# SeekStorm/SeekStorm

Measured on NVIDIA H100. Metric: queries/sec at top-10 (1M x 768 f32 cosine brute-force kNN), higher is better.
Workload: dtype f32

## Files before the change

seekstorm_b200/csrc/api.cu:

```cuda
#include <stdarg.h>
#include <string.h>
#include <algorithm>
#include <condition_variable>
#include <exception>
#include <memory>
#include <mutex>
#include <new>
#include <shared_mutex>
#include <vector>

#include "bm25.h"
#include "comm.h"
#include "common.cuh"
#include "vec_scan.h"

namespace ssb {

static thread_local char g_err[512] = "";

void set_error(const char* fmt, ...) {
    va_list ap; va_start(ap, fmt);
    vsnprintf(g_err, sizeof(g_err), fmt, ap);
    va_end(ap);
}
// ... 150 lines not shown
    const void* qsrc = queries;
    if (!is_device_ptr(queries)) {
        SSB_TRY(c.qstage.reserve(((size_t)nq * ix->dims + 3) / (queries_i8 ? 4 : 1) + 1, 0, st));
        SSB_CUDA_TRY(cudaMemcpyAsync(c.qstage.p, queries, qbytes, cudaMemcpyHostToDevice, st));
        c.stats.h2d_bytes += qbytes;
        qsrc = c.qstage.p;
    }
    if (scan == vec::Scan::I8_128) {
        SSB_TRY(c.q_i8.reserve((size_t)nq_pad * ix->dpad8, 0, st));
        if (queries_i8 && (ix->turbo || ix->cfg.vector_similarity != SSB_SIM_COSINE)) { set_error("int8 query codes are accepted for Cosine + ScalarQuantizationI8 only (the other quantisers need the query scale)"); return SSB_E_UNSUPPORTED; }
        if (ix->turbo) {
            SSB_TRY(c.q_scale.reserve(nq_pad, 0, st)); SSB_TRY(c.q_norm.reserve(nq_pad, 0, st));
            SSB_TRY(vec::launch_quantize_rows_turbo_i8((const float*)qsrc, ix->dims, nq, nq_pad, ix->dims, ix->tq_dim, ix->tq_mask, c.q_i8.p, ix->dpad8, c.q_scale.p,
                                                       c.q_norm.p, ix->cfg.vector_similarity == SSB_SIM_COSINE, ix->cfg.vector_similarity != SSB_SIM_EUCLIDEAN, st));
        } else if (ix->affine) {
            SSB_TRY(c.q_scale.reserve(nq_pad, 0, st)); SSB_TRY(c.q_norm.reserve(nq_pad, 0, st)); SSB_TRY(c.q_aff.reserve((size_t)nq_pad * 2, 0, st));
            SSB_TRY(vec::launch_quantize_rows_affine_i8((const float*)qsrc, ix->dims, nq, nq_pad, ix->dims, nullptr, nullptr, ix->aff_min, ix->aff_max, c.q_i8.p, ix->dpad8,
                                                        c.q_scale.p, c.q_norm.p, c.q_aff.p, 1, st));
        } else if (ix->cfg.vector_similarity != SSB_SIM_COSINE) {
            SSB_TRY(c.q_scale.reserve(nq_pad, 0, st)); SSB_TRY(c.q_norm.reserve(nq_pad, 0, st));
            SSB_TRY(vec::launch_quantize_rows_scale_i8((const float*)qsrc, ix->dims, nq, nq_pad, ix->dims, c.q_i8.p, ix->dpad8, c.q_scale.p, c.q_norm.p,
                                                       ix->cfg.vector_similarity == SSB_SIM_EUCLIDEAN, st));
        } else if (queries_i8) {
            SSB_CUDA_TRY(cudaMemsetAsync(c.q_i8.p, 0, (size_t)nq_pad * ix->dpad8, st));
            SSB_CUDA_TRY(cudaMemcpy2DAsync(c.q_i8.p, ix->dpad8, qsrc, ix->dims, ix->dims, nq, cudaMemcpyDeviceToDevice, st));
        } else {
            SSB_TRY(vec::launch_quantize_rows_i8((const float*)qsrc, ix->dims, nq, nq_pad, ix->dims, c.q_i8.p, ix->dpad8, st));
        }
    } else if (filter || scan == vec::Scan::Bf16_64 || scan == vec::Scan::Bf16_128 || scan == vec::Scan::Bf16_256) {
        SSB_TRY(c.qhi.reserve((size_t)nq_pad * ix->dpad, 0, st));
        SSB_TRY(c.qlo.reserve((size_t)nq_pad * ix->dpad, 0, st));
        if (filter) SSB_TRY(c.q_scale.reserve(nq_pad, 0, st));
        SSB_TRY(vec::launch_prep_split_queries_bf16((const float*)qsrc, nq, ix->dims, ix->dims, c.qhi.p, c.qlo.p, nq_pad, ix->dpad,
                                                    ix->cfg.vector_similarity == SSB_SIM_COSINE, st, (filter || ivf) ? c.qpad.p : nullptr,
                                                    filter ? c.q_scale.p : nullptr, filter ? ix->vec_err.p : nullptr));
    } else
    SSB_TRY(vec::launch_prep_queries((const float*)qsrc, nq, ix->dims, ix->dims, c.qpad.p, nq_pad, ix->dpad,
                                     ix->cfg.vector_similarity == SSB_SIM_COSINE, st));
    c.stats.kernel_launches += 1;
    if (ix->n_rows == 0) { SSB_CUDA_TRY(cudaMemsetAsync(keys_out_dev, 0, (size_t)nq * LIST * 8, st)); return SSB_OK; }
    size_t sb = vec::is_tensor_core(scan) ? vec::scan_tc_scratch_bytes(ix->n_sms, nq_pad) : vec::scan_scratch_bytes(ix->n_sms, nq_pad);
    const size_t head_words = sb / 8 + (size_t)nq_pad * LIST + (nq_pad + 1) / 2;
    SSB_TRY(c.scratch.reserve(head_words + (filter ? vec::refine_scratch_words(ix->n_sms, nq_pad) : 0), 0, st));
    vec::ScanArgs a{};
    a.rows = ix->rows.p; a.rows_hi = ix->rows_hi.p; a.rows_lo = ix->rows_lo.p; a.rows_h16 = ix->rows_h16.p; a.doc_ids = ix->doc_ids.p; a.n_rows = ix->n_rows; a.dpad = ix->dpad; a.queries_padded = c.qpad.p;
    a.nq_pad = nq_pad; a.nq_valid = nq; a.k = k; a.similarity = ix->cfg.vector_similarity; a.n_sms = ix->n_sms;
    a.scratch = c.scratch.p; a.scratch_bytes = sb;
    uint64_t* merged = c.scratch.p + sb / 8;
    a.keys_out = merged; a.ev0 = c.ev0; a.ev1 = c.ev1; c.ev_used = true;
    a.thr_buf = reinterpret_cast<uint32_t*>(merged + (size_t)nq_pad * LIST);
    a.ceil_keys = ceil_dev;
    if (ix->del.n) { a.del_slot = ix->del.d_slot; a.del_words = ix->del.d_words; }
    a.launches = &c.stats.kernel_launches;
    if (ivf) {
        vec::IvfArgs v{};
        v.medoids = ix->medoids.p; v.lvl_begin = ix->lvl_begin.p; v.cl_count = ix->cl_count.p;
        v.n_clusters = ix->n_clusters; v.n_levels = (uint32_t)ix->h_lvl_begin.size(); v.max_level_clusters = ix->max_level_clusters;
        v.queries_padded = c.qpad.p; v.nq = nq; v.nq_pad = nq_pad; v.dpad = ix->dpad; v.similarity = ix->cfg.vector_similarity;
        v.ann_mode = ivf->mode; v.n_probe = ivf->n_probe; v.cluster_threshold = ivf->thr;
        v.words = (ix->n_clusters + 31) / 32;
        SSB_TRY(c.ivf_scores.reserve((size_t)nq * ix->n_clusters, 0, st));
        SSB_TRY(c.ivf_sel.reserve((size_t)nq_pad * v.words, 0, st));
        SSB_TRY(c.ivf_obs.reserve(nq, 0, st));
        v.scores = c.ivf_scores.p; v.sel = c.ivf_sel.p; v.observed = c.ivf_obs.p; v.launches = &c.stats.kernel_launches;
        SSB_TRY(vec::launch_ivf_select(v, st));
        a.ivf_sel = c.ivf_sel.p; a.ivf_words = v.words; a.row_cluster = ix->row_cluster.p;
    }
    if (scan == vec::Scan::I8_128) {
        a.rows_i8 = ix->rows_i8.p; a.queries_i8 = c.q_i8.p; a.dpad8 = ix->dpad8;
        if (ix->turbo || ix->cfg.vector_similarity != SSB_SIM_COSINE) {
            a.i8_scaled = ix->cfg.vector_similarity == SSB_SIM_EUCLIDEAN ? (ix->affine ? 3 : 2) : 1;
            a.row_aff = ix->row_aff.p; a.q_aff = c.q_aff.p;
            a.row_scale = ix->row_scale.p; a.row_norm = ix->row_norm.p; a.q_scale = c.q_scale.p; a.q_norm = c.q_norm.p;
        }
    } else if (vec::is_tensor_core(scan)) {
        SSB_TRY(c.qhi.reserve((size_t)nq_pad * ix->dpad, 0, st));
        SSB_TRY(c.qlo.reserve((size_t)nq_pad * ix->dpad, 0, st));
        a.q_hi = c.qhi.p; a.q_lo = c.qlo.p;
        if (filter) a.q_scale = c.q_scale.p;
    }
    SSB_TRY(vec::is_tensor_core(scan) ? vec::launch_scan_tc(a, scan, st) : vec::launch_scan_ffma(a, st));
    if (filter) {
        vec::RefineArgs r{};
        r.rows = ix->rows.p; r.doc_ids = ix->doc_ids.p; r.n_rows = ix->n_rows; r.dpad = ix->dpad; r.queries_padded = c.qpad.p; r.margin = c.q_scale.p;
        r.keys = merged; r.keys_out = keys_out_dev;
        r.nq = nq; r.nq_pad = nq_pad; r.k = k;
        r.fb_lists = c.scratch.p + head_words;
        r.fb_state = reinterpret_cast<uint32_t*>(r.fb_lists + (size_t)nq_pad * ix->n_sms * LIST);
        r.del_slot = a.del_slot; r.del_words = a.del_words; r.ivf_sel = a.ivf_sel; r.ivf_words = a.ivf_words; r.row_cluster = a.row_cluster; r.n_sms = ix->n_sms; r.launches = &c.stats.kernel_launches;
        SSB_TRY(vec::launch_refine(r, st));
        c.fb_state = r.fb_state;
    } else {
        SSB_CUDA_TRY(cudaMemcpyAsync(keys_out_dev, merged, (size_t)nq * LIST * 8, cudaMemcpyDeviceToDevice, st));
    }
    const uint64_t pass_bytes = ix->n_rows * ix->dims * (scan == vec::Scan::I8_128 ? 1 : 4);
    c.stats.algorithmic_bytes += passes * pass_bytes;
    c.stats.scan_bytes_read += filter ? passes * pass_bytes / 2 + (uint64_t)nq * LIST * ix->dims * 4 : passes * pass_bytes;
    return SSB_OK;
}

uint32_t decode_list(const uint64_t* keys, uint32_t k, ssb_hit* hits, bool dedup) {
    uint32_t n = 0;
    for (uint32_t j = 0; j < LIST && n < k; j++) {
        const uint64_t key = keys[j];
        if (!key) break;
        const uint64_t doc = key_doc(key);
        if (dedup) { bool seen = false; for (uint32_t i = 0; i < n; i++) seen = seen || hits[i].doc_id == doc; if (seen) continue; }
        hits[n].doc_id = doc; hits[n].score = key_score(key); hits[n].pad = 0;
        n++;
    }
    return n;
}

void decode_keys(const uint64_t* keys, uint32_t nq, uint32_t k, ssb_hit* hits, uint32_t* n_hits, bool dedup = false) {
    for (uint32_t q = 0; q < nq; q++) {
        const uint32_t n = decode_list(keys + (size_t)q * LIST, k, hits + (size_t)q * k, dedup);
        for (uint32_t j = n; j < k; j++) { hits[(size_t)q * k + j].doc_id = 0; hits[(size_t)q * k + j].score = 0.f; hits[(size_t)q * k + j].pad = 0; }
        if (n_hits) n_hits[q] = n;
    }
}

int32_t shard_merge(ssb_index* ix, SearchCtx& c, uint64_t* keys_dev, uint32_t nq) {
    if (!ix->comm.active() || nq == 0) return SSB_OK;
    const size_t n = (size_t)nq * LIST;
    SSB_TRY(c.gather.reserve(n * ix->comm.world, 0, c.st));
    SSB_TRY(comm_all_gather_u64(ix->comm, keys_dev, c.gather.p, n, c.st));
    SSB_TRY(vec::launch_merge_lists(c.gather.p, ix->comm.world, nq, keys_dev, c.st));
    c.stats.kernel_launches += 2;
    return SSB_OK;
}
int32_t shard_sum_counts(ssb_index* ix, SearchCtx& c, uint64_t* counts_dev, uint32_t nq) {
    if (!ix->comm.active() || nq == 0 || !counts_dev) return SSB_OK;
    SSB_TRY(comm_all_reduce_sum_u64(ix->comm, counts_dev, nq, c.st));
    c.stats.kernel_launches += 1;
    return SSB_OK;
}

template <int W>
// ... 1031 lines not shown
```

seekstorm_b200/csrc/common.cuh:

```cuda
#pragma once
#include <cuda_runtime.h>
#include <cuda.h>
#include <stdint.h>
#include <stdio.h>
#include <string>

#include "../../include/seekstorm_b200.h"

namespace ssb {

void set_error(const char* fmt, ...);

#define SSB_CUDA_TRY(expr)                                                                   \
    do {                                                                                     \
        cudaError_t _e = (expr);                                                             \
        if (_e != cudaSuccess) {                                                             \
            ssb::set_error("%s:%d CUDA error %d (%s) in %s", __FILE__, __LINE__, (int)_e,   \
                           cudaGetErrorString(_e), #expr);                                   \
            return _e == cudaErrorMemoryAllocation ? SSB_E_NOMEM : SSB_E_CUDA;               \
        }                                                                                    \
    } while (0)

#define SSB_TRY(expr)                      \
    do {                                   \
// ... 21 lines not shown
#endif
}
__host__ __device__ __forceinline__ uint64_t pack_key(float score, uint32_t doc) {
    return ((uint64_t)ord_f32(score) << 32) | (uint64_t)(0xFFFFFFFFu - doc);
}
__host__ __device__ __forceinline__ uint32_t key_doc(uint64_t k) { return 0xFFFFFFFFu - (uint32_t)k; }
__host__ __device__ __forceinline__ float key_score(uint64_t k) { return unord_f32((uint32_t)(k >> 32)); }

#ifdef __CUDACC__
__device__ __forceinline__ uint64_t shfl64(uint64_t v, int src) {
    uint32_t lo = __shfl_sync(FULL, (uint32_t)v, src), hi = __shfl_sync(FULL, (uint32_t)(v >> 32), src);
    return ((uint64_t)hi << 32) | lo;
}
__device__ __forceinline__ uint64_t shfl64_up1(uint64_t v) {
    uint32_t lo = __shfl_up_sync(FULL, (uint32_t)v, 1), hi = __shfl_up_sync(FULL, (uint32_t)(v >> 32), 1);
    return ((uint64_t)hi << 32) | lo;
}
__device__ __forceinline__ uint64_t shfl64_xor(uint64_t v, int m) {
    uint32_t lo = __shfl_xor_sync(FULL, (uint32_t)v, m), hi = __shfl_xor_sync(FULL, (uint32_t)(v >> 32), m);
    return ((uint64_t)hi << 32) | lo;
}
__device__ __forceinline__ void wl_insert(uint64_t& L, uint64_t cand, int lane) {
    unsigned gt = __ballot_sync(FULL, L >= cand);
    int pos = __popc(gt);
    if (__any_sync(FULL, L == cand)) return;
    uint64_t up = shfl64_up1(L);
    if (lane == pos) L = cand;
    else if (lane > pos) L = up;
}
__device__ __forceinline__ uint64_t wl_sort_desc(uint64_t v, int lane) {
#pragma unroll
    for (int k = 2; k <= 32; k <<= 1) {
#pragma unroll
        for (int j = k >> 1; j > 0; j >>= 1) {
            const uint64_t p = shfl64_xor(v, j);
            const bool keep_max = ((lane & k) == 0) == ((lane & j) == 0);
            v = keep_max ? (v > p ? v : p) : (v < p ? v : p);
        }
    }
    return v;
}
__device__ __forceinline__ uint64_t wl_merge(uint64_t A, uint64_t B, int lane) {
    uint64_t Br = shfl64(B, 31 - lane);
    uint64_t M = A > Br ? A : Br;
#pragma unroll
    for (int s = 16; s >= 1; s >>= 1) {
        uint64_t P = shfl64_xor(M, s);
        bool keep_max = (lane & s) == 0;
        M = keep_max ? (M > P ? M : P) : (M < P ? M : P);
    }
    return M;
}

__device__ __forceinline__ bool doc_deleted(const uint32_t* __restrict__ del_slot, const uint64_t* __restrict__ del_words, uint32_t doc) {
    if (!del_slot) return false;
    const uint32_t slot = __ldg(&del_slot[doc >> 16]);
    if (slot == 0xFFFFFFFFu) return false;
    return ((__ldg(&del_words[(size_t)slot * 1024 + ((doc & 0xFFFFu) >> 6)]) >> (doc & 63u)) & 1ull) != 0;
}

__device__ __forceinline__ bool ivf_skipped(const uint32_t* __restrict__ sel, uint32_t words, uint32_t q, const uint32_t* __restrict__ row_cluster, uint32_t row) {
    if (!sel) return false;
    const uint32_t c = __ldg(&row_cluster[row]);
    return ((__ldg(&sel[(size_t)q * words + (c >> 5)]) >> (c & 31u)) & 1u) == 0u;
}

__device__ __forceinline__ uint32_t smem_u32(const void* p) { return (uint32_t)__cvta_generic_to_shared(p); }

__device__ __forceinline__ void mbar_init(uint64_t* bar, uint32_t count) {
    asm volatile("mbarrier.init.shared::cta.b64 [%0], %1;" ::"r"(smem_u32(bar)), "r"(count));
}
__device__ __forceinline__ void fence_mbar_init() {
    asm volatile("fence.mbarrier_init.release.cluster;" ::: "memory");
}
__device__ __forceinline__ void fence_proxy_async() {
    asm volatile("fence.proxy.async.shared::cta;" ::: "memory");
}
__device__ __forceinline__ void mbar_arrive_expect_tx(uint64_t* bar, uint32_t bytes) {
    asm volatile("mbarrier.arrive.expect_tx.shared::cta.b64 _, [%0], %1;" ::"r"(smem_u32(bar)), "r"(bytes)
                 : "memory");
}
__device__ __forceinline__ void mbar_arrive(uint64_t* bar) {
    asm volatile("mbarrier.arrive.shared::cta.b64 _, [%0];" ::"r"(smem_u32(bar)) : "memory");
}
__device__ __forceinline__ void mbar_wait(uint64_t* bar, uint32_t parity) {
    asm volatile(
        "{\n"
        ".reg .pred p;\n"
        "WAIT_LOOP:\n"
        "mbarrier.try_wait.parity.shared::cta.b64 p, [%0], %1;\n"
        "@p bra.uni WAIT_DONE;\n"
        "bra.uni WAIT_LOOP;\n"
        "WAIT_DONE:\n"
        "}\n" ::"r"(smem_u32(bar)),
        "r"(parity)
        : "memory");
}
__device__ __forceinline__ void tma_load_2d(void* dst, const CUtensorMap* map, int c0, int c1, uint64_t* bar) {
    asm volatile(
        "cp.async.bulk.tensor.2d.shared::cluster.global.mbarrier::complete_tx::bytes [%0], [%1, {%3, %4}], [%2];"
        ::"r"(smem_u32(dst)), "l"(map), "r"(smem_u32(bar)), "r"(c0), "r"(c1)
        : "memory");
}
__device__ __forceinline__ void tma_prefetch_desc(const CUtensorMap* map) {
    asm volatile("prefetch.tensormap [%0];" ::"l"(map) : "memory");
}
// ... 9 lines not shown
```

seekstorm_b200/csrc/vec_refine.cu:

```cuda
#include "common.cuh"
#include "vec_scan.h"

namespace ssb {
namespace vec {
namespace rf {

constexpr int RTHREADS = 128;
constexpr int QF = 4;
constexpr int FTHREADS = 256;

__device__ __forceinline__ float dot4(const float4 a, const float4 b, float s) {
    s = fmaf(a.x, b.x, s); s = fmaf(a.y, b.y, s); s = fmaf(a.z, b.z, s); return fmaf(a.w, b.w, s);
}

__global__ void __launch_bounds__(RTHREADS)
refine_candidates(const float* __restrict__ rows, const uint32_t* __restrict__ doc_ids, uint32_t dpad, const float* __restrict__ queries,
                  const float* __restrict__ margin, const uint64_t* keys, uint64_t* keys_out, uint32_t k, uint32_t* __restrict__ fb_state) {
    __shared__ uint64_t ex[LIST];
    const int warp = threadIdx.x >> 5, lane = threadIdx.x & 31;
    const uint32_t q = blockIdx.x;
    const uint64_t mine = keys[(size_t)q * LIST + lane];
    const float* qv = queries + (size_t)q * dpad;
    uint64_t ck[8]; const float* rp[8]; float s[8];
#pragma unroll
    for (int c = 0; c < 8; c++) {
        ck[c] = shfl64(mine, warp * 8 + c);
        rp[c] = rows + (size_t)(ck[c] ? key_doc(ck[c]) : 0u) * dpad;
        s[c] = 0.f;
    }
    if (ck[0]) {
        for (uint32_t i = lane * 4; i < dpad; i += 128) {
            const float4 b = *reinterpret_cast<const float4*>(qv + i);
#pragma unroll
            for (int c = 0; c < 8; c++) s[c] = dot4(__ldg(reinterpret_cast<const float4*>(rp[c] + i)), b, s[c]);
        }
    }
#pragma unroll
    for (int c = 0; c < 8; c++) {
        float v = s[c];
        for (int m = 16; m; m >>= 1) v += __shfl_xor_sync(FULL, v, m);
        if (lane == 0) {
            uint64_t key = 0;
            if (ck[c] && v == v) { const uint32_t row = key_doc(ck[c]); key = pack_key(v, doc_ids ? __ldg(&doc_ids[row]) : row); }
            ex[warp * 8 + c] = key;
        }
    }
    __syncthreads();
    if (warp == 0) {
        keys_out[(size_t)q * LIST + lane] = wl_sort_desc(ex[lane], lane);
        const uint64_t kth = shfl64(mine, (int)k - 1), last = shfl64(mine, LIST - 1);
        if (lane == 0 && last && kth) {
            const float m = margin[q], th = __fsub_rd(key_score(kth), m);
            if (!(m == m) || key_score(last) >= th) fb_state[1 + atomicAdd(&fb_state[0], 1u)] = q;
        }
    }
}

__global__ void __launch_bounds__(FTHREADS)
fallback_scan(const float* __restrict__ rows, const uint32_t* __restrict__ doc_ids, uint64_t n_rows, uint32_t dpad,
              const float* __restrict__ queries, const uint32_t* __restrict__ fb_state, uint64_t* __restrict__ fb_lists ,
              uint32_t k, const uint32_t* __restrict__ del_slot, const uint64_t* __restrict__ del_words,
              const uint32_t* __restrict__ ivf_sel, uint32_t ivf_words, const uint32_t* __restrict__ row_cluster) {
    const uint32_t nf = fb_state[0];
    if (nf == 0) return;
    extern __shared__ __align__(16) float qs[];
    __shared__ uint64_t sm[FTHREADS / 32][QF][LIST];
    const int warp = threadIdx.x >> 5, lane = threadIdx.x & 31;
    for (uint32_t base = 0; base < nf; base += QF) {
        for (uint32_t i = threadIdx.x; i < QF * dpad; i += FTHREADS) {
            const uint32_t j = i / dpad;
            qs[i] = base + j < nf ? queries[(size_t)fb_state[1 + base + j] * dpad + (i - j * dpad)] : 0.f;
        }
        __syncthreads();
        uint64_t L[QF];
#pragma unroll
        for (int j = 0; j < QF; j++) L[j] = 0;
        for (uint64_t row = (uint64_t)blockIdx.x * (FTHREADS / 32) + warp; row < n_rows; row += (uint64_t)gridDim.x * (FTHREADS / 32)) {
            float s[QF];
#pragma unroll
            for (int j = 0; j < QF; j++) s[j] = 0.f;
            const float* r = rows + row * dpad;
            for (uint32_t i = lane * 4; i < dpad; i += 128) {
                const float4 a = __ldg(reinterpret_cast<const float4*>(r + i));
#pragma unroll
                for (int j = 0; j < QF; j++) s[j] = dot4(a, *reinterpret_cast<const float4*>(qs + j * dpad + i), s[j]);
            }
#pragma unroll
            for (int j = 0; j < QF; j++) for (int m = 16; m; m >>= 1) s[j] += __shfl_xor_sync(FULL, s[j], m);
            const uint32_t doc = doc_ids ? __ldg(&doc_ids[row]) : (uint32_t)row;
            if (doc_deleted(del_slot, del_words, doc)) continue;
#pragma unroll
            for (int j = 0; j < QF; j++) {
                if (!(s[j] == s[j]) || base + j >= nf) continue;
                if (ivf_skipped(ivf_sel, ivf_words, fb_state[1 + base + j], row_cluster, (uint32_t)row)) continue;
                const uint64_t key = pack_key(s[j], doc);
                if (key > shfl64(L[j], (int)k - 1)) wl_insert(L[j], key, lane);
            }
        }
#pragma unroll
        for (int j = 0; j < QF; j++) sm[warp][j][lane] = L[j];
        __syncthreads();
        if (warp < QF && base + warp < nf) {
            uint64_t M = sm[0][warp][lane];
            for (int w = 1; w < FTHREADS / 32; w++) M = wl_merge(M, sm[w][warp][lane], lane);
            fb_lists[((size_t)(base + warp) * gridDim.x + blockIdx.x) * LIST + lane] = M;
        }
        __syncthreads();
    }
}

__global__ void __launch_bounds__(32)
fallback_merge(const uint32_t* __restrict__ fb_state, const uint64_t* __restrict__ fb_lists, uint32_t n_lists, uint64_t* __restrict__ keys) {
    const uint32_t nf = fb_state[0];
    const int lane = threadIdx.x;
    for (uint32_t slot = blockIdx.x; slot < nf; slot += gridDim.x) {
        uint64_t L = 0;
        for (uint32_t l = 0; l < n_lists; l++) {
            const uint64_t B = fb_lists[((size_t)slot * n_lists + l) * LIST + lane];
            if (__any_sync(FULL, B != 0)) L = wl_merge(L, B, lane);
        }
        keys[(size_t)fb_state[1 + slot] * LIST + lane] = L;
    }
}

}

size_t refine_scratch_words(int n_sms, uint32_t nq_pad) { return (size_t)nq_pad * (size_t)n_sms * LIST + (nq_pad + 2) / 2 + 1; }

int32_t launch_refine(const RefineArgs& a, cudaStream_t st) {
    if (a.nq == 0) return SSB_OK;
    SSB_CUDA_TRY(cudaMemsetAsync(a.fb_state, 0, 4, st));
    rf::refine_candidates<<<a.nq, rf::RTHREADS, 0, st>>>(a.rows, a.doc_ids, a.dpad, a.queries_padded, a.margin, a.keys, a.keys_out, a.k, a.fb_state);
    SSB_CUDA_TRY(cudaGetLastError());
    const int smem = rf::QF * (int)a.dpad * 4;
    if (smem > 200 * 1024) { set_error("filter scan: vector_dims too large for the fallback scan"); return SSB_E_UNSUPPORTED; }
    if (smem > 40 * 1024) SSB_CUDA_TRY(cudaFuncSetAttribute(rf::fallback_scan, cudaFuncAttributeMaxDynamicSharedMemorySize, smem));
    rf::fallback_scan<<<a.n_sms, rf::FTHREADS, smem, st>>>(a.rows, a.doc_ids, a.n_rows, a.dpad, a.queries_padded, a.fb_state, a.fb_lists, a.k,
                                                           a.del_slot, a.del_words, a.ivf_sel, a.ivf_words, a.row_cluster);
    SSB_CUDA_TRY(cudaGetLastError());
    rf::fallback_merge<<<64, 32, 0, st>>>(a.fb_state, a.fb_lists, (uint32_t)a.n_sms, a.keys_out);
    SSB_CUDA_TRY(cudaGetLastError());
    if (a.launches) *a.launches += 3;
    return SSB_OK;
}

}
}
```

seekstorm_b200/csrc/vec_scan.cu:

```cuda
#include <limits.h>
#include "common.cuh"
#include "vec_scan.h"

namespace ssb {
namespace vec {

constexpr int KC = 32;
constexpr int TILE_ROWS = 512;
constexpr int BOX_ROWS = 256;
constexpr int QT = (int)queries_per_pass(Scan::Ffma);
constexpr int STAGES = 3;
constexpr int CWARPS = 8;
constexpr int THREADS = (CWARPS + 1) * 32;
constexpr int A_BYTES = TILE_ROWS * KC * 4;
constexpr int Q_BYTES = QT * KC * 4;
constexpr int STAGE_TX = A_BYTES + Q_BYTES;
constexpr int LISTS_BYTES = CWARPS * 8 * LIST * 8;
constexpr int SMEM_BYTES = STAGES * (A_BYTES + Q_BYTES) + LISTS_BYTES + 2 * STAGES * 8;

__device__ __forceinline__ void ffma2(float2& c, float2 a, float2 b) {
    c.x = __fmaf_rn(a.x, b.x, c.x);
    c.y = __fmaf_rn(a.y, b.y, c.y);
}
__device__ __forceinline__ float2 fsub2(float2 a, float2 b) { return make_float2(__fsub_rn(a.x, b.x), __fsub_rn(a.y, b.y)); }
// ... 104 lines not shown
                                const uint64_t key = ((uint64_t)so << 32) | (uint64_t)(0xFFFFFFFFu - (doc_ids ? __ldg(&doc_ids[row]) : row));
                                if (key >= __ldg(&ceil_keys[group * QT + qh + q])) so = 0u;
                            }
                            const uint32_t mx = __reduce_max_sync(FULL, so);
                            if (lane == j * 8 + q) keep = mx;
                        }
                    }
                    uint32_t* gmax = (uint32_t*)scratch;
                    gmax[(size_t)(group * QT + qh + (lane & 7)) * (n_tiles * 16) + (tile * 16 + rg * 4 + (lane >> 3))] = keep;
                    continue;
                }
                if (kc + 1 == n_kchunks) {
#pragma unroll
                    for (int j = 0; j < 4; j++) {
                        uint32_t row = tile * TILE_ROWS + (uint32_t)r0 + 32u * j;
                        bool valid = row < n_rows;
#pragma unroll
                        for (int q = 0; q < 8; q++) {
                            float sum = acc[j][q].x + acc[j][q].y;
                            float sc = (SIM == SSB_SIM_EUCLIDEAN) ? -sum : sum;
                            acc[j][q] = make_float2(0.f, 0.f);
                            uint32_t so = ord_f32(sc);
                            unsigned m = __ballot_sync(FULL, valid && so >= thr[q] && sc == sc);
                            if (m) {
                                const uint64_t ceil = ceil_keys ? __ldg(&ceil_keys[group * QT + qh + q]) : ~0ull;
                                uint64_t Lq = myL[q * LIST];
                                while (m) {
                                    int src = __ffs(m) - 1;
                                    m &= m - 1;
                                    uint32_t so_s = __shfl_sync(FULL, so, src);
                                    uint32_t row_s = __shfl_sync(FULL, row, src);
                                    uint32_t doc = doc_ids ? __ldg(&doc_ids[row_s]) : row_s;
                                    uint64_t key = ((uint64_t)so_s << 32) | (uint64_t)(0xFFFFFFFFu - doc);
                                    if (key < ceil && !doc_deleted(del_slot, del_words, doc) && !ivf_skipped(ivf_sel, ivf_words, group * QT + qh + q, row_cluster, row_s))
                                        wl_insert(Lq, key, lane);
                                }
                                myL[q * LIST] = Lq;
                                const uint32_t kth = (uint32_t)(shfl64(Lq, (int)k - 1) >> 32);
                                if (kth > thr[q]) thr[q] = kth;
                            }
                        }
                    }
                }
            }
        }
        if (sample_mode) return;
        const uint32_t n_lists = gridDim.x * (CWARPS / 2);
        uint64_t* out = scratch + ((size_t)group * n_lists + (size_t)blockIdx.x * (CWARPS / 2) + rg) * QT * LIST;
#pragma unroll
        for (int q = 0; q < 8; q++) out[(qh + q) * LIST + lane] = myL[q * LIST];
    }
}

constexpr uint32_t MERGE_MAX_LISTS = 2048;
__global__ void __launch_bounds__(256)
merge_lists(const uint64_t* __restrict__ in, uint32_t n_lists, uint32_t qt, uint64_t* __restrict__ out ) {
    __shared__ uint64_t sm[8][LIST];
    __shared__ uint16_t ne[MERGE_MAX_LISTS];
    __shared__ uint32_t n_ne;
    const int warp = threadIdx.x >> 5, lane = threadIdx.x & 31;
    const uint32_t q = blockIdx.x;
    const uint64_t* base = in + (size_t)(q / qt) * n_lists * qt * LIST + (size_t)(q % qt) * LIST;
    if (threadIdx.x == 0) n_ne = 0;
    __syncthreads();
    const bool small = n_lists <= MERGE_MAX_LISTS;
    if (small) {
        for (uint32_t l = threadIdx.x; l < n_lists; l += 256)
            if (__ldg(&base[(size_t)l * qt * LIST]) != 0ull) ne[atomicAdd(&n_ne, 1u)] = (uint16_t)l;
        __syncthreads();
    }
    const uint32_t cnt = small ? n_ne : n_lists;
    uint64_t L = 0;
    for (uint32_t i = warp; i < cnt; i += 32) {
        uint64_t B[4];
#pragma unroll
        for (int u = 0; u < 4; u++) {
            const uint32_t k = i + 8 * u;
            B[u] = k < cnt ? __ldg(&base[(size_t)(small ? (uint32_t)ne[k] : k) * qt * LIST + lane]) : 0ull;
        }
#pragma unroll
        for (int u = 0; u < 4; u++) if (__any_sync(FULL, B[u] != 0)) L = wl_merge(L, B[u], lane);
    }
    sm[warp][lane] = L;
    __syncthreads();
    if (warp == 0) {
        for (int w = 1; w < 8; w++) L = wl_merge(L, sm[w][lane], lane);
        out[(size_t)q * LIST + lane] = L;
    }
}

__global__ void prep_queries(const float* __restrict__ q, uint32_t nq, uint32_t dims, uint64_t qstride,
                             float* __restrict__ out, uint32_t nq_pad, uint32_t dpad, int normalize) {
    const int lane = threadIdx.x & 31;
    uint32_t row = blockIdx.x * (blockDim.x >> 5) + (threadIdx.x >> 5);
    if (row >= nq_pad) return;
    float* o = out + (size_t)row * dpad;
    if (row >= nq) { for (uint32_t i = lane; i < dpad; i += 32) o[i] = 0.f; return; }
    const float* src = q + (size_t)row * qstride;
    float f = 1.f;
    if (normalize) {
        float s = 0.f;
        for (uint32_t i = lane; i < dims; i += 32) { float v = src[i]; s = fmaf(v, v, s); }
        for (int m = 16; m; m >>= 1) s += __shfl_xor_sync(FULL, s, m);
        f = 1.0f / sqrtf(s);
    }
    for (uint32_t i = lane; i < dpad; i += 32) o[i] = i < dims ? src[i] * f : 0.f;
}

__global__ void normalize_rows(float* __restrict__ rows, uint64_t n, uint32_t dims, uint32_t dpad, int normalize) {
    const int lane = threadIdx.x & 31;
    uint64_t row = (uint64_t)blockIdx.x * (blockDim.x >> 5) + (threadIdx.x >> 5);
    if (row >= n) return;
    float* r = rows + row * dpad;
    float f = 1.f;
    if (normalize) {
        float s = 0.f;
        for (uint32_t i = lane; i < dims; i += 32) { float v = r[i]; s = fmaf(v, v, s); }
        for (int m = 16; m; m >>= 1) s += __shfl_xor_sync(FULL, s, m);
        f = 1.0f / sqrtf(s);
    }
    for (uint32_t i = lane; i < dpad; i += 32) r[i] = i < dims ? r[i] * f : 0.f;
}

__global__ void quantize_rows_i8(const float* __restrict__ src, uint64_t src_stride, uint64_t n, uint64_t n_out, uint32_t dims,
                                 int8_t* __restrict__ dst, uint32_t dpad8) {
    const int lane = threadIdx.x & 31;
    const uint64_t row = (uint64_t)blockIdx.x * (blockDim.x >> 5) + (threadIdx.x >> 5);
    if (row >= n_out) return;
    int8_t* o = dst + row * dpad8;
    if (row >= n) { for (uint32_t i = lane; i < dpad8; i += 32) o[i] = 0; return; }
    const float* r = src + row * src_stride;
    float s = 0.0f;
    for (uint32_t base = 0; base < dims; base += 32) {
        const float v = base + lane < dims ? r[base + lane] : 0.0f;
        const float p = __fmul_rn(v, v);
#pragma unroll
        for (int l = 0; l < 32; l++) s = __fadd_rn(s, __shfl_sync(FULL, p, l));
    }
    const float f = __fdiv_rn(1.0f, __fsqrt_rn(s));
    for (uint32_t i = lane; i < dpad8; i += 32) {
        int8_t q = 0;
// ... 303 lines not shown
```

seekstorm_b200/csrc/vec_scan.h:

```cpp
#pragma once
#include <cuda_runtime.h>
#include <stdint.h>

#include "common.cuh"
#include "scan_plan.h"

namespace ssb {
namespace vec {

struct ScanArgs {
    const float* rows;
    const void* rows_hi = nullptr; const void* rows_lo = nullptr;
    const void* rows_h16 = nullptr;
    const uint32_t* doc_ids;
    uint64_t n_rows;
    uint32_t dpad;
    const float* queries_padded;
    uint32_t nq_pad;
    uint32_t nq_valid = 0;
    uint32_t k;
    uint32_t similarity;
    int n_sms;
    uint64_t* scratch;
    size_t scratch_bytes;
    uint64_t* keys_out;
    cudaEvent_t ev0 = nullptr, ev1 = nullptr;
    float* q_hi = nullptr; float* q_lo = nullptr;
    uint32_t* thr_buf = nullptr;
    const uint32_t* thr_init = nullptr;
    const uint64_t* ceil_keys = nullptr;
    uint64_t* launches = nullptr;
    const int8_t* rows_i8 = nullptr;
    const int8_t* queries_i8 = nullptr;
    uint32_t dpad8 = 0;
    int i8_scaled = 0;
    const float* row_scale = nullptr; const float* row_norm = nullptr;
    const float* q_scale = nullptr; const float* q_norm = nullptr;
    const int* row_aff = nullptr; const int* q_aff = nullptr;
    const uint32_t* del_slot = nullptr; const uint64_t* del_words = nullptr;
    bool sample_groupmax = false;
    const uint32_t* ivf_sel = nullptr; uint32_t ivf_words = 0; const uint32_t* row_cluster = nullptr;
};

template <class F>
int32_t with_threshold_seed(const ScanArgs& a, uint64_t sample_rows, F launch) {
    if (a.thr_init || !a.thr_buf || a.del_slot || a.ivf_sel || a.n_rows < 65536) return launch(a);
    ScanArgs pre = a;
    pre.n_rows = sample_rows; pre.ev0 = nullptr; pre.ev1 = nullptr;
    pre.sample_groupmax = true;
    SSB_TRY(launch(pre));
    ScanArgs full = a;
    full.thr_init = a.thr_buf;
    return launch(full);
}

int32_t launch_scan_ffma(const ScanArgs& a, cudaStream_t st);
size_t scan_scratch_bytes(int n_sms, uint32_t nq_pad);
int32_t launch_scan_tc(const ScanArgs& a, Scan s , cudaStream_t st);
size_t scan_tc_scratch_bytes(int n_sms, uint32_t nq_pad);
int32_t launch_prep_split_queries_bf16(const float* q, uint32_t nq, uint32_t dims, uint64_t qstride, void* hi, void* lo, uint32_t nq_pad,
                                       uint32_t dpad, int normalize, cudaStream_t st, float* f32_out = nullptr, float* margin_out = nullptr,
                                       const uint32_t* row_err = nullptr);
int32_t launch_rows_f16_err(const float* rows, void* h16, uint64_t n, uint32_t dpad, float scale, uint32_t* err, cudaStream_t st);
int32_t launch_max_abs_f32(const float* x, size_t n, uint32_t* out_bits, cudaStream_t st);
struct RefineArgs {
    const float* rows; const uint32_t* doc_ids; uint64_t n_rows; uint32_t dpad;
    const float* queries_padded;
    const float* margin;
    const uint64_t* keys;
    uint64_t* keys_out;
    uint32_t nq, nq_pad, k;
    uint32_t* fb_state;
    uint64_t* fb_lists;
    const uint32_t* del_slot; const uint64_t* del_words;
    const uint32_t* ivf_sel; uint32_t ivf_words; const uint32_t* row_cluster;
    int n_sms;
    uint64_t* launches;
};
struct IvfArgs {
    const float* medoids;
    const uint32_t* lvl_begin;
    const uint32_t* cl_count;
    uint32_t n_clusters, n_levels, max_level_clusters;
    const float* queries_padded;
    uint32_t nq, nq_pad, dpad, similarity;
    uint32_t ann_mode, n_probe; float cluster_threshold;
    float* scores;
    uint32_t* sel; uint32_t words;
    uint64_t* observed;
    uint64_t* launches;
};
int32_t launch_ivf_select(const IvfArgs& a, cudaStream_t st);
int32_t launch_gather_rows(const float* src, const uint32_t* idx_dev, uint32_t n, uint32_t dpad, float* dst, cudaStream_t st);
int32_t launch_refine(const RefineArgs& a, cudaStream_t st);
size_t refine_scratch_words(int n_sms, uint32_t nq_pad);
int32_t launch_split_rows_bf16(const float* rows, void* hi, void* lo, size_t n_elems, cudaStream_t st);
void launch_kth_from_groupmax(const void* gmax, uint32_t n_groups, uint32_t nq, uint32_t k, uint32_t* thr, int is_int, cudaStream_t st);
void merge_lists_generic(const uint64_t* in, uint32_t n_lists, uint32_t qt, uint32_t nq, uint64_t* out, cudaStream_t st);
int32_t launch_prep_queries(const float* q, uint32_t nq, uint32_t dims, uint64_t qstride, float* out,
                            uint32_t nq_pad, uint32_t dpad, int normalize, cudaStream_t st);
int32_t launch_quantize_rows_i8(const float* src, uint64_t src_stride, uint64_t n, uint64_t n_out, uint32_t dims, int8_t* dst,
                                uint32_t dpad8, cudaStream_t st);
int32_t launch_quantize_rows_scale_i8(const float* src, uint64_t src_stride, uint64_t n, uint64_t n_out, uint32_t dims, int8_t* dst,
                                      uint32_t dpad8, float* scale_out, float* norm_out, int want_norm, cudaStream_t st);
int32_t launch_rows_minmax(const float* src, uint64_t src_stride, uint64_t n, uint32_t dims, float* minmax_out, cudaStream_t st);
int32_t launch_quantize_rows_affine_i8(const float* src, uint64_t src_stride, uint64_t n, uint64_t n_out, uint32_t dims, const float* scale_in, const int* zp_in,
                                       float st_min, float st_max, int8_t* dst, uint32_t dpad8, float* scale_out, float* norm_out, int* aff_out, int is_query,
                                       cudaStream_t st);
void affine_walk_rows(const float* minmax, uint64_t n, float* st_min, float* st_max, float* scale_out, int* zp_out);
int32_t launch_quantize_rows_turbo_i8(const float* src, uint64_t src_stride, uint64_t n, uint64_t n_out, uint32_t dims, uint32_t tq_dim, const float* mask,
                                      int8_t* dst, uint32_t dpad8, float* scale_out, float* norm_out, int normalize, int negate, cudaStream_t st);
int32_t launch_normalize_rows(float* rows, uint64_t n, uint32_t dims, uint32_t dpad, int normalize, cudaStream_t st);
int32_t launch_fill_doc_ids(uint32_t* out, const uint16_t* local_ids, uint32_t level_id, uint32_t n, cudaStream_t st);
int32_t launch_merge_lists(const uint64_t* in, uint32_t n_lists, uint32_t nq, uint64_t* out, cudaStream_t st);

}
}
```

seekstorm_b200/csrc/vec_scan_tc.cu:

```cuda
#include <cuda_bf16.h>
#include <stdlib.h>
#include <type_traits>
#include <cuda_fp16.h>

#include "common.cuh"
#include "vec_scan.h"

namespace ssb {
namespace vec {

namespace tc {
constexpr int KC = 32;
constexpr int TM = 128;
constexpr int MT = 2;
constexpr int TROWS = TM * MT;
constexpr int A1_BYTES = TM * KC * 4;
constexpr int THREADS = 384;
constexpr int CHUNK = 8;
constexpr int XB_STRIDE = CHUNK + 1;
constexpr int REC_WORDS = 32 * XB_STRIDE;
constexpr int XB_BYTES = 8 * REC_WORDS * 4;
constexpr int QSLOTS = 26;
constexpr int QUEUE_BYTES = QSLOTS * REC_WORDS * 4 + (3 * QSLOTS + 2) * 4;
constexpr int SMEM_MAX = 232448;
// ... 384 lines not shown
                            mma<PREC, NQH>(acc[m], a_hi + am + o, b_hi + o, (kc | kk) != 0);
                            mma<PREC, NQH>(acc[m], a_lo + am + o, b_hi + o, 1);
                            mma<PREC, NQH>(acc[m], a_hi + am + o, b_lo + o, 1);
                        }
                    }
                } else {
                    const uint64_t a1 = gmma_desc_k64(sa + C::ALO_OFF), a2 = gmma_desc_k64(sa + C::A2_OFF);
                    const uint64_t b1 = gmma_desc_k64(sb), b2 = gmma_desc_k64(sb + C::B_BYTES);
#pragma unroll
                    for (int m = 0; m < MW; m++) {
                        const uint64_t am = (uint64_t)((m * 64 * 64) >> 4);
#pragma unroll
                        for (uint32_t kk = 0; kk < 2; kk++) {
                            const uint64_t o = (uint64_t)(kk * 2);
                            mma<PREC, NQH>(acc[m], a1 + am + o, b1 + o, (kc | kk) != 0);
                            mma<PREC, NQH>(acc[m], a2 + am + o, b1 + o, 1);
                            mma<PREC, NQH>(acc[m], a1 + am + o, b2 + o, 1);
                        }
                    }
                }
                wg_commit();
                wg_wait<1>();
                if (kc > 0 && lane == 0) {
                    const uint32_t sp = (it - 1) % STAGES;
                    mbar_arrive(&empty[sp]);
                    if (PAIR) mbar_arrive_cta(&empty[sp], rank ^ 1u);
                }
            }
            wg_wait<0>();
            if (lane == 0) {
                const uint32_t sp = (it - 1) % STAGES;
                mbar_arrive(&empty[sp]);
                if (PAIR) mbar_arrive_cta(&empty[sp], rank ^ 1u);
            }
#pragma unroll
            for (int m = 0; m < MW; m++)
#pragma unroll
                for (int i = 0; i < NQH / 2; i++) fence_reg(acc[m][i]);

#pragma unroll
            for (int p = 0; p < MW / 2; p++) {
                const uint32_t row = tile * TROWS + (uint32_t)(64 * (2 * p + (lane >> 4)) + 16 * w + (lane & 15));
                const bool valid = row < n_rows;
                float rs = 0.f, rn = 0.f;
                int2 ra = make_int2(0, 0);
                if (SCALED) {
                    rs = valid ? __ldg(&row_scale[row]) : 0.f;
                    rn = (SCALED >= 2 && valid) ? __ldg(&row_norm[row]) : 0.f;
                    ra = (SCALED == 3 && valid) ? __ldg(&row_aff[row]) : make_int2(0, 0);
                }
#pragma unroll
                for (int jb = 0; jb < NQH / CHUNK; jb++) {
                    const int c = q0 / CHUNK + jb;
                    if (FRAG_VOTE && !sample_mode) {
                        const uint2 t = *reinterpret_cast<const uint2*>(thr_u + c * CHUNK + 2 * (lane & 3));
                        const float t0 = unord_f32(max(t.x, ORD_NEG_INF)), t1 = unord_f32(max(t.y, ORD_NEG_INF));
                        bool any = false;
#pragma unroll
                        for (int hm = 0; hm < 2; hm++)
#pragma unroll
                            for (int h = 0; h < 2; h++)
                                any |= (acc[2 * p + hm][4 * jb + 2 * h] >= t0) | (acc[2 * p + hm][4 * jb + 2 * h + 1] >= t1);
                        if (!__any_sync(FULL, any)) continue;
                    }
                    if (QUEUE) {
                        int s;
                        for (;;) {
                            unsigned fr = __ballot_sync(FULL, lane < QSLOTS && qstate[lane] == 0u);
                            int got = -1;
                            if (lane == 0)
                                while (fr) {
                                    const int i = __ffs(fr) - 1; fr &= fr - 1;
                                    if (atomicCAS((uint32_t*)&qstate[i], 0u, 1u) == 0u) { got = i; break; }
                                }
                            s = __shfl_sync(FULL, got, 0);
                            if (s >= 0) break;
                            __nanosleep(64);
                        }
                        uint32_t* rec = xbuf + s * REC_WORDS;
#pragma unroll
                        for (int hm = 0; hm < 2; hm++)
#pragma unroll
                            for (int h = 0; h < 2; h++) {
                                uint32_t* d = rec + (hm * 16 + (lane >> 2) + 8 * h) * XB_STRIDE + 2 * (lane & 3);
                                xb_put(&d[0], acc[2 * p + hm][4 * jb + 2 * h]);
                                xb_put(&d[1], acc[2 * p + hm][4 * jb + 2 * h + 1]);
                            }
                        if (lane == 0) { qmeta[2 * s] = tile; qmeta[2 * s + 1] = (uint32_t)w; }
                        __threadfence_block();
                        __syncwarp();
                        if (lane == 0) qstate[s] = 2u + (uint32_t)c;
                        continue;
                    }
                    __syncwarp();
#pragma unroll
                    for (int hm = 0; hm < 2; hm++)
#pragma unroll
                        for (int h = 0; h < 2; h++) {
                            uint32_t* d = xb + (hm * 16 + (lane >> 2) + 8 * h) * XB_STRIDE + 2 * (lane & 3);
                            xb_put(&d[0], acc[2 * p + hm][4 * jb + 2 * h]);
                            xb_put(&d[1], acc[2 * p + hm][4 * jb + 2 * h + 1]);
                        }
                    __syncwarp();
                    uint32_t v[CHUNK];
#pragma unroll
                    for (int j = 0; j < CHUNK; j++) {
// ... 198 lines not shown
        if (!a.thr_init) tc::split_queries_tf32<<<(unsigned)((nel + 255) / 256), 256, 0, st>>>(a.queries_padded, a.q_hi, a.q_lo, nel);
    } else if constexpr (PREC == tc::PREC_F16F) {
        if (!a.rows_h16 || !a.q_scale) { set_error("tensor-core filter scan: the index holds no fp16 plane / no margins"); return SSB_E_STATE; }
        SSB_TRY(encode_tmap_2d(&tmA, a.rows_h16, 2 , a.dpad, a.n_rows, (uint64_t)a.dpad * 2, 64, C::TROWS, 128));
        SSB_TRY(encode_tmap_2d(&tmBh, a.q_hi, 2, a.dpad, a.nq_pad, (uint64_t)a.dpad * 2, 64, PAIR ? NQ / 2 : NQ, 128));
        tmBl = tmBh; tmA2 = tmA;
        n_kchunks = (a.dpad + 63) / 64;
    } else {
        if (!a.rows_hi || !a.rows_lo) { set_error("tensor-core bf16 scan: the index holds no bf16 planes"); return SSB_E_STATE; }
        SSB_TRY(encode_tmap_2d(&tmA, a.rows_hi, 2 , a.dpad, a.n_rows, (uint64_t)a.dpad * 2, tc::KC, C::TROWS, 64));
        SSB_TRY(encode_tmap_2d(&tmA2, a.rows_lo, 2 , a.dpad, a.n_rows, (uint64_t)a.dpad * 2, tc::KC, C::TROWS, 64));
        SSB_TRY(encode_tmap_2d(&tmBh, a.q_hi, 2 , a.dpad, a.nq_pad, (uint64_t)a.dpad * 2, tc::KC, NQ, 64));
        SSB_TRY(encode_tmap_2d(&tmBl, a.q_lo, 2 , a.dpad, a.nq_pad, (uint64_t)a.dpad * 2, tc::KC, NQ, 64));
    }
    uint32_t gx = n_tiles < (uint32_t)a.n_sms ? n_tiles : (uint32_t)a.n_sms;
    if (PAIR) {
        uint32_t n_pairs = (n_tiles + 1) / 2, n_clusters = (uint32_t)a.n_sms / 2;
        gx = 2 * (n_pairs < n_clusters ? n_pairs : n_clusters);
    }
    const bool queue = NQ == 256 && a.thr_init && !a.sample_groupmax && !a.del_slot && !a.ivf_sel;
    using CQ = tc::Cfg<NQ, PREC, BRES, NQ == 256>;
    const uint32_t n_lists = queue ? 1u : 4u;
    if ((size_t)n_groups * gx * n_lists * NQ * LIST * 8 > a.scratch_bytes) { set_error("vector scan scratch too small"); return SSB_E_STATE; }
    uint32_t nst = queue ? CQ::STAGES : C::STAGES;
    int smem = queue ? CQ::SMEM : C::SMEM;
    if (BRES) {
        const int fixed = (int)n_kchunks * C::B_BYTES + C::FIXED;
        nst = (uint32_t)((tc::SMEM_MAX - fixed) / C::STAGE_BYTES);
        if (nst > (uint32_t)tc::MAX_STAGES) nst = tc::MAX_STAGES;
        smem = fixed + (int)nst * C::STAGE_BYTES;
    }
    auto kern = queue ? tc::scan_tc<NQ, PREC, BRES, SCALED, PAIR, NQ == 256> : tc::scan_tc<NQ, PREC, BRES, SCALED, PAIR, false>;
    SSB_CUDA_TRY(cudaFuncSetAttribute(kern, cudaFuncAttributeMaxDynamicSharedMemorySize, BRES ? tc::SMEM_MAX : smem));
    cudaLaunchConfig_t cfg{};
    cfg.gridDim = dim3(gx, n_groups); cfg.blockDim = dim3(tc::THREADS); cfg.dynamicSmemBytes = (size_t)smem; cfg.stream = st;
    cudaLaunchAttribute at[1];
    at[0].id = cudaLaunchAttributeClusterDimension; at[0].val.clusterDim.x = PAIR ? 2 : 1; at[0].val.clusterDim.y = 1; at[0].val.clusterDim.z = 1;
    cfg.attrs = at; cfg.numAttrs = PAIR ? 1 : 0;
    if (a.ev0) cudaEventRecord(a.ev0, st);
    SSB_CUDA_TRY(cudaLaunchKernelEx(&cfg, kern, tmA, tmA2, tmBh, tmBl, (uint32_t)a.n_rows, n_kchunks, n_tiles,
                                    a.k, a.doc_ids, a.scratch, a.thr_init, a.nq_valid ? a.nq_valid : a.nq_pad, a.ceil_keys, nst,
                                    a.del_slot, a.del_words, a.row_scale, a.row_norm, a.q_scale, a.q_norm,
                                    (const int2*)a.row_aff, (const int2*)a.q_aff,
                                    PREC == tc::PREC_I8 ? nullptr : a.ivf_sel, a.ivf_words, a.row_cluster,
                                    a.sample_groupmax ? 1u : 0u));
    if (a.ev1) cudaEventRecord(a.ev1, st);
    if (a.sample_groupmax) {
        tc::kth_from_groupmax<<<a.nq_pad, 256, 0, st>>>((const int*)a.scratch, n_tiles * (C::TROWS / 32), a.nq_pad, a.k, a.thr_buf,
                                                        0, PREC == tc::PREC_F16F ? a.q_scale : nullptr);
        SSB_CUDA_TRY(cudaGetLastError());
        if (a.launches) *a.launches += PREC == tc::PREC_TF32 ? 3 : 2;
        return SSB_OK;
    }
    merge_lists_generic(a.scratch, gx * n_lists, NQ, a.nq_pad, a.keys_out, st);
    SSB_CUDA_TRY(cudaGetLastError());
    if (a.launches) *a.launches += 2;
    return SSB_OK;
}

static int32_t launch_scan_tc_impl(const ScanArgs& a, Scan s, cudaStream_t st) {
    if (a.n_rows == 0 || a.nq_pad == 0) return SSB_OK;
    if (a.nq_pad % queries_per_pass(s) != 0) { set_error("tensor-core scan: query count must be padded to the %u-query tile", queries_per_pass(s)); return SSB_E_INVALID; }
    if (s != Scan::I8_128 && a.similarity == SSB_SIM_EUCLIDEAN) { set_error("tensor-core scan supports Dot/Cosine only"); return SSB_E_UNSUPPORTED; }
    switch (s) {
    case Scan::Tf32_64: return launch_tc_n<64, tc::PREC_TF32>(a, st);
    case Scan::Tf32_128: return launch_tc_n<128, tc::PREC_TF32>(a, st);
    case Scan::Bf16_64: return launch_tc_n<64, tc::PREC_BF16>(a, st);
    case Scan::Bf16_128: return launch_tc_n<128, tc::PREC_BF16>(a, st);
    case Scan::Bf16_256: return launch_tc_n<256, tc::PREC_BF16>(a, st);
    case Scan::F16f_128: return launch_tc_n<128, tc::PREC_F16F>(a, st);
    case Scan::F16f_256: return launch_tc_n<256, tc::PREC_F16F>(a, st);
    case Scan::F16f_256Pair:
        return a.sample_groupmax ? launch_tc_n<256, tc::PREC_F16F>(a, st) : launch_tc_n<256, tc::PREC_F16F, false, 0, true>(a, st);
    case Scan::I8_128: {
        if (!a.rows_i8 || !a.queries_i8 || a.dpad8 % 128) { set_error("int8 scan: bad arguments"); return SSB_E_INVALID; }
        const bool res = tc::i8_resident(a.dpad8);
        if (a.i8_scaled) {
            if (!a.row_scale || !a.q_scale || (a.i8_scaled >= 2 && (!a.row_norm || !a.q_norm)) || (a.i8_scaled == 3 && (!a.row_aff || !a.q_aff))) { set_error("scaled int8 scan: missing scale / norm arrays"); return SSB_E_INVALID; }
            if (a.i8_scaled == 3) return res ? launch_tc_n<128, tc::PREC_I8, true, 3>(a, st) : launch_tc_n<128, tc::PREC_I8, false, 3>(a, st);
            if (a.i8_scaled == 1) return res ? launch_tc_n<128, tc::PREC_I8, true, 1>(a, st) : launch_tc_n<128, tc::PREC_I8, false, 1>(a, st);
            return res ? launch_tc_n<128, tc::PREC_I8, true, 2>(a, st) : launch_tc_n<128, tc::PREC_I8, false, 2>(a, st);
        }
        return res ? launch_tc_n<128, tc::PREC_I8, true>(a, st) : launch_tc_n<128, tc::PREC_I8, false>(a, st);
    }
    case Scan::Ffma: break;
    }
    set_error("tensor-core scan: the FP32 scan is launch_scan_ffma"); return SSB_E_INVALID;
}

int32_t launch_scan_tc(const ScanArgs& a, Scan s, cudaStream_t st) {
    const uint64_t trows = queries_per_pass(s) == 256 ? 128 : tc::TROWS;
    static const int env_tiles = [] { const char* e = getenv("SSB_TC_SAMPLE_TILES"); return e ? atoi(e) : 0; }();
    const int sample_tiles = env_tiles > 0 ? (env_tiles > 16 ? 16 : env_tiles) : ((s == Scan::F16f_256 || s == Scan::F16f_256Pair) ? 2 : 1);
    uint64_t rows = (uint64_t)a.n_sms * trows * sample_tiles;
    if (rows > a.n_rows / 4) rows = a.n_rows / 4 / trows * trows;
    return with_threshold_seed(a, rows, [s, st](const ScanArgs& x) { return launch_scan_tc_impl(x, s, st); });
}

void launch_kth_from_groupmax(const void* gmax, uint32_t n_groups, uint32_t nq, uint32_t k, uint32_t* thr, int is_int, cudaStream_t st) {
    if (nq) tc::kth_from_groupmax<<<nq, 256, 0, st>>>((const int*)gmax, n_groups, nq, k, thr, is_int, nullptr);
}

int32_t launch_prep_split_queries_bf16(const float* q, uint32_t nq, uint32_t dims, uint64_t qstride, void* hi, void* lo, uint32_t nq_pad,
                                       uint32_t dpad, int normalize, cudaStream_t st, float* f32_out, float* margin_out, const uint32_t* row_err) {
    if (nq_pad == 0) return SSB_OK;
    tc::prep_split_queries_bf16<<<(nq_pad + 7) / 8, 256, 0, st>>>(q, nq, dims, qstride, (__nv_bfloat16*)hi, (__nv_bfloat16*)lo, nq_pad, dpad, normalize,
// ... 30 lines not shown
```

Before: 264,900.

## Fuse per-list merge into refine kernel and add sample-mode groupmax path

Result: faster. 296,200, median of 6 (+11.8%).

```diff
diff --git a/seekstorm_b200/csrc/api.cu b/seekstorm_b200/csrc/api.cu
--- a/seekstorm_b200/csrc/api.cu
+++ b/seekstorm_b200/csrc/api.cu
@@ -226,6 +226,8 @@
     a.ceil_keys = ceil_dev;
     if (ix->del.n) { a.del_slot = ix->del.d_slot; a.del_words = ix->del.d_words; }
     a.launches = &c.stats.kernel_launches;
+    uint32_t unmerged = 0;
+    if (filter) a.unmerged_lists = &unmerged;
     if (ivf) {
         vec::IvfArgs v{};
         v.medoids = ix->medoids.p; v.lvl_begin = ix->lvl_begin.p; v.cl_count = ix->cl_count.p;
@@ -258,6 +260,7 @@
         vec::RefineArgs r{};
         r.rows = ix->rows.p; r.doc_ids = ix->doc_ids.p; r.n_rows = ix->n_rows; r.dpad = ix->dpad; r.queries_padded = c.qpad.p; r.margin = c.q_scale.p;
         r.keys = merged; r.keys_out = keys_out_dev;
+        if (unmerged) { r.lists = a.scratch; r.n_lists = unmerged; r.qt = vec::queries_per_pass(scan); }
         r.nq = nq; r.nq_pad = nq_pad; r.k = k;
         r.fb_lists = c.scratch.p + head_words;
         r.fb_state = reinterpret_cast<uint32_t*>(r.fb_lists + (size_t)nq_pad * ix->n_sms * LIST);
diff --git a/seekstorm_b200/csrc/common.cuh b/seekstorm_b200/csrc/common.cuh
--- a/seekstorm_b200/csrc/common.cuh
+++ b/seekstorm_b200/csrc/common.cuh
@@ -97,6 +97,41 @@
     return M;
 }
 
+constexpr uint32_t MERGE_MAX_LISTS = 2048;
+struct MergeSmem {
+    uint64_t part[8][LIST];
+    uint16_t ne[MERGE_MAX_LISTS];
+    uint32_t n_ne;
+};
+__device__ __forceinline__ uint64_t merge_lists_block(const uint64_t* __restrict__ base, uint32_t n_lists, size_t stride, MergeSmem& sm) {
+    const int warp = threadIdx.x >> 5, lane = threadIdx.x & 31;
+    if (threadIdx.x == 0) sm.n_ne = 0;
+    __syncthreads();
+    const bool small = n_lists <= MERGE_MAX_LISTS;
+    if (small) {
+        for (uint32_t l = threadIdx.x; l < n_lists; l += 256)
+            if (__ldg(&base[(size_t)l * stride]) != 0ull) sm.ne[atomicAdd(&sm.n_ne, 1u)] = (uint16_t)l;
+        __syncthreads();
+    }
+    const uint32_t cnt = small ? sm.n_ne : n_lists;
+    uint64_t L = 0;
+    for (uint32_t i = warp; i < cnt; i += 32) {
+        uint64_t B[4];
+#pragma unroll
+        for (int u = 0; u < 4; u++) {
+            const uint32_t k = i + 8 * u;
+            B[u] = k < cnt ? __ldg(&base[(size_t)(small ? (uint32_t)sm.ne[k] : k) * stride + lane]) : 0ull;
+        }
+#pragma unroll
+        for (int u = 0; u < 4; u++) if (__any_sync(FULL, B[u] != 0)) L = wl_merge(L, B[u], lane);
+    }
+    sm.part[warp][lane] = L;
+    __syncthreads();
+    L = sm.part[0][lane];
+    for (int w = 1; w < 8; w++) L = wl_merge(L, sm.part[w][lane], lane);
+    return L;
+}
+
 __device__ __forceinline__ bool doc_deleted(const uint32_t* __restrict__ del_slot, const uint64_t* __restrict__ del_words, uint32_t doc) {
     if (!del_slot) return false;
     const uint32_t slot = __ldg(&del_slot[doc >> 16]);
diff --git a/seekstorm_b200/csrc/vec_refine.cu b/seekstorm_b200/csrc/vec_refine.cu
--- a/seekstorm_b200/csrc/vec_refine.cu
+++ b/seekstorm_b200/csrc/vec_refine.cu
@@ -5,7 +5,8 @@
 namespace vec {
 namespace rf {
 
-constexpr int RTHREADS = 128;
+constexpr int RTHREADS = 256;
+constexpr int RCAND = LIST / (RTHREADS / 32);
 constexpr int QF = 4;
 constexpr int FTHREADS = 256;
 
@@ -15,16 +16,19 @@
 
 __global__ void __launch_bounds__(RTHREADS)
 refine_candidates(const float* __restrict__ rows, const uint32_t* __restrict__ doc_ids, uint32_t dpad, const float* __restrict__ queries,
-                  const float* __restrict__ margin, const uint64_t* keys, uint64_t* keys_out, uint32_t k, uint32_t* __restrict__ fb_state) {
+                  const float* __restrict__ margin, const uint64_t* keys, const uint64_t* __restrict__ lists, uint32_t n_lists, uint32_t qt,
+                  uint64_t* keys_out, uint32_t k, uint32_t* __restrict__ fb_state) {
     __shared__ uint64_t ex[LIST];
+    __shared__ MergeSmem msm;
     const int warp = threadIdx.x >> 5, lane = threadIdx.x & 31;
     const uint32_t q = blockIdx.x;
-    const uint64_t mine = keys[(size_t)q * LIST + lane];
+    const uint64_t mine = lists ? merge_lists_block(lists + (size_t)(q / qt) * n_lists * qt * LIST + (size_t)(q % qt) * LIST, n_lists, (size_t)qt * LIST, msm)
+                                : keys[(size_t)q * LIST + lane];
     const float* qv = queries + (size_t)q * dpad;
-    uint64_t ck[8]; const float* rp[8]; float s[8];
+    uint64_t ck[RCAND]; const float* rp[RCAND]; float s[RCAND];
 #pragma unroll
-    for (int c = 0; c < 8; c++) {
-        ck[c] = shfl64(mine, warp * 8 + c);
+    for (int c = 0; c < RCAND; c++) {
+        ck[c] = shfl64(mine, warp * RCAND + c);
         rp[c] = rows + (size_t)(ck[c] ? key_doc(ck[c]) : 0u) * dpad;
         s[c] = 0.f;
     }
@@ -32,17 +36,17 @@
         for (uint32_t i = lane * 4; i < dpad; i += 128) {
             const float4 b = *reinterpret_cast<const float4*>(qv + i);
 #pragma unroll
-            for (int c = 0; c < 8; c++) s[c] = dot4(__ldg(reinterpret_cast<const float4*>(rp[c] + i)), b, s[c]);
+            for (int c = 0; c < RCAND; c++) s[c] = dot4(__ldg(reinterpret_cast<const float4*>(rp[c] + i)), b, s[c]);
         }
     }
 #pragma unroll
-    for (int c = 0; c < 8; c++) {
+    for (int c = 0; c < RCAND; c++) {
         float v = s[c];
         for (int m = 16; m; m >>= 1) v += __shfl_xor_sync(FULL, v, m);
         if (lane == 0) {
             uint64_t key = 0;
             if (ck[c] && v == v) { const uint32_t row = key_doc(ck[c]); key = pack_key(v, doc_ids ? __ldg(&doc_ids[row]) : row); }
-            ex[warp * 8 + c] = key;
+            ex[warp * RCAND + c] = key;
         }
     }
     __syncthreads();
@@ -130,7 +134,8 @@
 int32_t launch_refine(const RefineArgs& a, cudaStream_t st) {
     if (a.nq == 0) return SSB_OK;
     SSB_CUDA_TRY(cudaMemsetAsync(a.fb_state, 0, 4, st));
-    rf::refine_candidates<<<a.nq, rf::RTHREADS, 0, st>>>(a.rows, a.doc_ids, a.dpad, a.queries_padded, a.margin, a.keys, a.keys_out, a.k, a.fb_state);
+    rf::refine_candidates<<<a.nq, rf::RTHREADS, 0, st>>>(a.rows, a.doc_ids, a.dpad, a.queries_padded, a.margin, a.keys, a.lists, a.n_lists, a.qt,
+                                                         a.keys_out, a.k, a.fb_state);
     SSB_CUDA_TRY(cudaGetLastError());
     const int smem = rf::QF * (int)a.dpad * 4;
     if (smem > 200 * 1024) { set_error("filter scan: vector_dims too large for the fallback scan"); return SSB_E_UNSUPPORTED; }
diff --git a/seekstorm_b200/csrc/vec_scan.cu b/seekstorm_b200/csrc/vec_scan.cu
--- a/seekstorm_b200/csrc/vec_scan.cu
+++ b/seekstorm_b200/csrc/vec_scan.cu
@@ -180,41 +180,12 @@
     }
 }
 
-constexpr uint32_t MERGE_MAX_LISTS = 2048;
 __global__ void __launch_bounds__(256)
 merge_lists(const uint64_t* __restrict__ in, uint32_t n_lists, uint32_t qt, uint64_t* __restrict__ out ) {
-    __shared__ uint64_t sm[8][LIST];
-    __shared__ uint16_t ne[MERGE_MAX_LISTS];
-    __shared__ uint32_t n_ne;
-    const int warp = threadIdx.x >> 5, lane = threadIdx.x & 31;
+    __shared__ MergeSmem sm;
     const uint32_t q = blockIdx.x;
-    const uint64_t* base = in + (size_t)(q / qt) * n_lists * qt * LIST + (size_t)(q % qt) * LIST;
-    if (threadIdx.x == 0) n_ne = 0;
-    __syncthreads();
-    const bool small = n_lists <= MERGE_MAX_LISTS;
-    if (small) {
-        for (uint32_t l = threadIdx.x; l < n_lists; l += 256)
-            if (__ldg(&base[(size_t)l * qt * LIST]) != 0ull) ne[atomicAdd(&n_ne, 1u)] = (uint16_t)l;
-        __syncthreads();
-    }
-    const uint32_t cnt = small ? n_ne : n_lists;
-    uint64_t L = 0;
-    for (uint32_t i = warp; i < cnt; i += 32) {
-        uint64_t B[4];
-#pragma unroll
-        for (int u = 0; u < 4; u++) {
-            const uint32_t k = i + 8 * u;
-            B[u] = k < cnt ? __ldg(&base[(size_t)(small ? (uint32_t)ne[k] : k) * qt * LIST + lane]) : 0ull;
-        }
-#pragma unroll
-        for (int u = 0; u < 4; u++) if (__any_sync(FULL, B[u] != 0)) L = wl_merge(L, B[u], lane);
-    }
-    sm[warp][lane] = L;
-    __syncthreads();
-    if (warp == 0) {
-        for (int w = 1; w < 8; w++) L = wl_merge(L, sm[w][lane], lane);
-        out[(size_t)q * LIST + lane] = L;
-    }
+    const uint64_t L = merge_lists_block(in + (size_t)(q / qt) * n_lists * qt * LIST + (size_t)(q % qt) * LIST, n_lists, (size_t)qt * LIST, sm);
+    if (threadIdx.x < 32) out[(size_t)q * LIST + threadIdx.x] = L;
 }
 
 __global__ void prep_queries(const float* __restrict__ q, uint32_t nq, uint32_t dims, uint64_t qstride,
diff --git a/seekstorm_b200/csrc/vec_scan.h b/seekstorm_b200/csrc/vec_scan.h
--- a/seekstorm_b200/csrc/vec_scan.h
+++ b/seekstorm_b200/csrc/vec_scan.h
@@ -40,6 +40,7 @@
     const uint32_t* del_slot = nullptr; const uint64_t* del_words = nullptr;
     bool sample_groupmax = false;
     const uint32_t* ivf_sel = nullptr; uint32_t ivf_words = 0; const uint32_t* row_cluster = nullptr;
+    uint32_t* unmerged_lists = nullptr;
 };
 
 template <class F>
@@ -68,6 +69,8 @@
     const float* queries_padded;
     const float* margin;
     const uint64_t* keys;
+    const uint64_t* lists = nullptr;
+    uint32_t n_lists = 0, qt = 0;
     uint64_t* keys_out;
     uint32_t nq, nq_pad, k;
     uint32_t* fb_state;
diff --git a/seekstorm_b200/csrc/vec_scan_tc.cu b/seekstorm_b200/csrc/vec_scan_tc.cu
--- a/seekstorm_b200/csrc/vec_scan_tc.cu
+++ b/seekstorm_b200/csrc/vec_scan_tc.cu
@@ -460,6 +460,31 @@
 #pragma unroll
                 for (int jb = 0; jb < NQH / CHUNK; jb++) {
                     const int c = q0 / CHUNK + jb;
+                    if constexpr (FRAG_VOTE && !QUEUE) if (sample_mode) {
+                        uint32_t mx[2] = {0u, 0u};
+#pragma unroll
+                        for (int hm = 0; hm < 2; hm++)
+#pragma unroll
+                            for (int h = 0; h < 2; h++)
+#pragma unroll
+                                for (int b = 0; b < 2; b++) {
+                                    const uint32_t r = tile * TROWS + (uint32_t)(64 * (2 * p + hm) + 16 * w + (lane >> 2) + 8 * h);
+                                    const float sc = acc[2 * p + hm][4 * jb + 2 * h + b];
+                                    uint32_t so = (r < n_rows && sc == sc) ? ord_f32(sc) : 0u;
+                                    if (ceil_keys && so) {
+                                        const uint64_t key = ((uint64_t)so << 32) | (uint64_t)(0xFFFFFFFFu - (doc_ids ? __ldg(&doc_ids[r]) : r));
+                                        if (key >= __ldg(&ceil_keys[blockIdx.y * NQ + c * CHUNK + 2 * (lane & 3) + b])) so = 0u;
+                                    }
+                                    mx[b] = max(mx[b], so);
+                                }
+#pragma unroll
+                        for (int m = 4; m < 32; m <<= 1) { mx[0] = max(mx[0], __shfl_xor_sync(FULL, mx[0], m)); mx[1] = max(mx[1], __shfl_xor_sync(FULL, mx[1], m)); }
+                        if (lane < 4) {
+                            uint32_t* g = gmaxu + (size_t)(blockIdx.y * NQ + c * CHUNK + 2 * lane) * n_rg + (tile * (TROWS / 32) + p * 4 + w);
+                            g[0] = mx[0]; g[n_rg] = mx[1];
+                        }
+                        continue;
+                    }
                     if (FRAG_VOTE && !sample_mode) {
                         const uint2 t = *reinterpret_cast<const uint2*>(thr_u + c * CHUNK + 2 * (lane & 3));
                         const float t0 = unord_f32(max(t.x, ORD_NEG_INF)), t1 = unord_f32(max(t.y, ORD_NEG_INF));
@@ -764,6 +789,11 @@
         if (a.launches) *a.launches += PREC == tc::PREC_TF32 ? 3 : 2;
         return SSB_OK;
     }
+    if (PREC == tc::PREC_F16F && queue && a.unmerged_lists) {
+        *a.unmerged_lists = gx;
+        if (a.launches) *a.launches += 1;
+        return SSB_OK;
+    }
     merge_lists_generic(a.scratch, gx * n_lists, NQ, a.nq_pad, a.keys_out, st);
     SSB_CUDA_TRY(cudaGetLastError());
     if (a.launches) *a.launches += 2;
```
